# jnvance/DMRG.x

Hardware: NVIDIA B200
Metric: superblock H*psi algorithmic GB/s (higher is better)
Workload: dtype f64

## Files before the change

### dmrg.x_b200/csrc/dev_cuda.cu

```cuda
#include <cuda_runtime.h>
#include <dlfcn.h>
#include <nccl.h>

#include <chrono>
#include <map>
#include <unordered_map>
#include <cstdio>
#include <cstring>
#include <algorithm>
#include <stdexcept>
#include <string>
#include <vector>

#include "dev.h"

namespace dev {

static thread_local std::string g_err;
static long long g_launches = 0;
const char* last_error() { return g_err.c_str(); }
long long launch_count() { return g_launches; }

#define CUDA_OK(call)                                                                                   \
    do {                                                                                                \
        cudaError_t e_ = (call);                                                                        \
        if (e_ != cudaSuccess) {                                                                        \
            char buf_[512];                                                                             \
            snprintf(buf_, sizeof buf_, "%s failed at %s:%d: %s", #call, __FILE__, __LINE__, cudaGetErrorString(e_)); \
            g_err = buf_;                                                                               \
            fprintf(stderr, "[dmrgx] %s\n", buf_);                                                      \
            throw std::runtime_error(buf_);                                                             \
        }                                                                                               \
    } while (0)

struct Stream {
    int device = 0;
    cudaStream_t s = nullptr;
    bool own = false;
    double* partials = nullptr;
    unsigned int* ticket = nullptr;
    int num_sms = 148;
    struct Arena { char* base = nullptr; size_t size = 0; std::map<size_t, size_t> free;  };
    std::vector<Arena> arenas;
    std::unordered_map<void*, size_t> live;
    size_t bytes_reserved = 0, bytes_free = 0, bytes_live = 0, bytes_live_peak = 0;
    double malloc_seconds = 0;
    long long malloc_calls = 0;
    ncclComm_t comm = nullptr;
    int rank = 0, world = 1;
    int spmm_smem = 0;
    bool chain_cfg = false;
    bool gram_cfg = false;
    bool gram_rect_cfg = false;
    cudaStream_t aux = nullptr;
    cudaEvent_t ev_fork = nullptr, ev_join = nullptr;
};

constexpr int RED_BLOCKS = 592;
constexpr int RED_MAXVEC = 40;

int init(int device, void* user_stream, Stream** out) {
    try {
        int ndev = 0;
        cudaError_t e = cudaGetDeviceCount(&ndev);
        if (e != cudaSuccess || ndev == 0) {
            g_err = std::string("no CUDA device: ") + cudaGetErrorString(e) + " — dmrgx has no CPU path";
            return 100;
        }
        CUDA_OK(cudaSetDevice(device));
        Stream* st = new Stream();
        st->device = device;
        if (user_stream) { st->s = (cudaStream_t)user_stream; st->own = false; }
        else { CUDA_OK(cudaStreamCreateWithFlags(&st->s, cudaStreamNonBlocking)); st->own = true; }
        cudaDeviceProp prop;
        CUDA_OK(cudaGetDeviceProperties(&prop, device));
        st->num_sms = prop.multiProcessorCount;
        CUDA_OK(cudaMalloc(&st->partials, sizeof(double) * RED_BLOCKS * RED_MAXVEC));
        CUDA_OK(cudaMalloc(&st->ticket, sizeof(unsigned int)));
        CUDA_OK(cudaMemset(st->ticket, 0, sizeof(unsigned int)));
        *out = st;
        return 0;
    } catch (const std::exception&) { return 100; }
}

static void comm_destroy_(Stream* st);
void destroy(Stream* st) {
    if (!st) return;
    cudaSetDevice(st->device);
    cudaStreamSynchronize(st->s);
    if (getenv("DMRGX_TRACE") || getenv("DMRGX_ALLOC_STATS"))
        fprintf(stderr, "[trace] allocator: %lld cudaMalloc calls, %.3f s, %.2f GB reserved, peak in use %.2f GB\n", st->malloc_calls, st->malloc_seconds,
                st->bytes_reserved / 1e9, st->bytes_live_peak / 1e9);
    if (st->comm) comm_destroy_(st);
    if (st->aux) cudaStreamDestroy(st->aux);
    if (st->ev_fork) cudaEventDestroy(st->ev_fork);
    if (st->ev_join) cudaEventDestroy(st->ev_join);
    for (auto& ar : st->arenas) cudaFree(ar.base);
    cudaFree(st->partials);
    cudaFree(st->ticket);
    if (st->own) cudaStreamDestroy(st->s);
    delete st;
}
void make_current(Stream* st) { cudaSetDevice(st->device); }

constexpr size_t HEAP_SLAB = (size_t)1 << 30, HEAP_GRAIN = (size_t)256 << 20;
static void heap_add_arena(Stream* st, void* slab, size_t sz) {
    Stream::Arena ar; ar.base = (char*)slab; ar.size = sz; ar.free[0] = sz;
    st->arenas.push_back(ar); st->bytes_reserved += sz; st->bytes_free += sz;
}
void* malloc_bytes(Stream* st, size_t bytes) {
    const size_t need = (std::max<size_t>(bytes, 1) + 511) & ~(size_t)511;
    for (;;) {
        Stream::Arena* best_a = nullptr;
        std::map<size_t, size_t>::iterator best;
        size_t best_len = ~(size_t)0;
        for (auto& ar : st->arenas)
            for (auto f = ar.free.begin(); f != ar.free.end(); ++f)
                if (f->second >= need && f->second < best_len) { best_a = &ar; best = f; best_len = f->second; if (best_len == need) break; }
        if (best_a) {
            const size_t off = best->first, len = best->second;
            best_a->free.erase(best);
            if (len > need) best_a->free[off + need] = len - need;
            void* p = best_a->base + off;
            st->live[p] = need;
            st->bytes_free -= need; st->bytes_live += need;
            if (st->bytes_live > st->bytes_live_peak) st->bytes_live_peak = st->bytes_live;
            return p;
        }
        const size_t quarter = std::min(HEAP_SLAB * 8, st->bytes_reserved / 4 / HEAP_GRAIN * HEAP_GRAIN);
        const size_t sz = std::max(std::max(HEAP_SLAB, quarter), (need + HEAP_GRAIN - 1) / HEAP_GRAIN * HEAP_GRAIN);
        void* slab = nullptr;
        const auto t0 = std::chrono::steady_clock::now();
        cudaError_t e = cudaMalloc(&slab, sz);
        if (e != cudaSuccess) {
            cudaGetLastError();
            CUDA_OK(cudaStreamSynchronize(st->s));
            for (size_t i = 0; i < st->arenas.size();) {
                Stream::Arena& ar = st->arenas[i];
                if (ar.free.size() == 1 && ar.free.begin()->second == ar.size) {
                    cudaFree(ar.base); st->bytes_reserved -= ar.size; st->bytes_free -= ar.size; st->arenas.erase(st->arenas.begin() + (long)i);
                } else ++i;
            }
            e = cudaMalloc(&slab, need);
            if (e == cudaSuccess) heap_add_arena(st, slab, need);
        } else heap_add_arena(st, slab, sz);
        st->malloc_seconds += std::chrono::duration<double>(std::chrono::steady_clock::now() - t0).count();
        st->malloc_calls++;
        CUDA_OK(e);
    }
}
void free_bytes(Stream* st, void* p) {
    if (!p) return;
    auto f = st->live.find(p);
    if (f == st->live.end()) return;
    size_t len = f->second;
    st->live.erase(f);
    st->bytes_free += len; st->bytes_live -= len;
    for (auto& ar : st->arenas) {
        if ((char*)p < ar.base || (char*)p >= ar.base + ar.size) continue;
        size_t off = (size_t)((char*)p - ar.base);
        auto nx = ar.free.lower_bound(off);
        if (nx != ar.free.end() && off + len == nx->first) { len += nx->second; nx = ar.free.erase(nx); }
        if (nx != ar.free.begin()) {
            auto pv = std::prev(nx);
            if (pv->first + pv->second == off) { pv->second += len; return; }
        }
        ar.free[off] = len;
        return;
    }
}
void h2d(Stream* st, void* dst, const void* src, size_t bytes) { if (bytes) CUDA_OK(cudaMemcpyAsync(dst, src, bytes, cudaMemcpyHostToDevice, st->s)); }
void d2h(Stream* st, void* dst, const void* src, size_t bytes) { if (bytes) CUDA_OK(cudaMemcpyAsync(dst, src, bytes, cudaMemcpyDeviceToHost, st->s)); }
void d2d(Stream* st, void* dst, const void* src, size_t bytes) { if (bytes) CUDA_OK(cudaMemcpyAsync(dst, src, bytes, cudaMemcpyDeviceToDevice, st->s)); }
void memset0(Stream* st, void* dst, size_t bytes) { if (bytes) CUDA_OK(cudaMemsetAsync(dst, 0, bytes, st->s)); }
void sync(Stream* st) { CUDA_OK(cudaStreamSynchronize(st->s)); }

#define LAUNCH_CHECK() do { ++g_launches; CUDA_OK(cudaGetLastError()); } while (0)

constexpr int BM = 64, BK = 16, NTHREADS = 128;
constexpr int S_MK = BK + 4;
constexpr int S_KM = BM + 4;
constexpr int SMEM_TILE = (BM * S_MK > BK * S_KM) ? BM * S_MK : BK * S_KM;

__device__ __forceinline__ void cp_async8(double* smem_dst, const double* gsrc, bool valid) {
    unsigned s = (unsigned)__cvta_generic_to_shared(smem_dst);
    int sz = valid ? 8 : 0;
    asm volatile("cp.async.ca.shared.global [%0], [%1], 8, %2;\n" ::"r"(s), "l"(gsrc), "r"(sz));
}
__device__ __forceinline__ void cp_async8_all(double* smem_dst, const double* gsrc) {
    unsigned s = (unsigned)__cvta_generic_to_shared(smem_dst);
    asm volatile("cp.async.ca.shared.global [%0], [%1], 8;\n" ::"r"(s), "l"(gsrc));
}
__device__ __forceinline__ void cp_async_commit() { asm volatile("cp.async.commit_group;\n" ::); }
template <int N>
__device__ __forceinline__ void cp_async_wait() { asm volatile("cp.async.wait_group %0;\n" ::"n"(N)); }

__device__ __forceinline__ void dmma_m8n8k4(double& c0, double& c1, double a, double b) {
    asm volatile("mma.sync.aligned.m8n8k4.row.col.f64.f64.f64.f64 {%0,%1}, {%2}, {%3}, {%0,%1};\n"
                 : "+d"(c0), "+d"(c1)
                 : "d"(a), "d"(b));
}

template <bool MK>
struct Stager {
    const double* base;
    int off[8];
    long long kstep;
    int soff;
    int k0;
    unsigned rowmask;
    static constexpr int SI = MK ? 8 * S_MK : 2 * S_KM;
    __device__ __forceinline__ void init(const double* b, long long ld_row, long long ld_k, int ext, int tid) {
        base = b;
        if (MK) {
            const int k = tid & 15, r0 = tid >> 4;
            rowmask = 0;
#pragma unroll
            for (int i = 0; i < 8; ++i) {
                int r = r0 + 8 * i;
                if (r < ext) rowmask |= 1u << i;
                r = r < ext ? r : ext - 1;
                off[i] = (int)(r * ld_row + k * ld_k);
            }
            soff = r0 * S_MK + k;
            k0 = k;
        } else {
            const int r = tid & 63, kk = tid >> 6;
            const int rc = r < ext ? r : ext - 1;
            rowmask = r < ext ? 0xffu : 0u;
#pragma unroll
            for (int i = 0; i < 8; ++i) off[i] = (int)(rc * ld_row + (kk + 2 * i) * ld_k);
            soff = kk * S_KM + r;
            k0 = kk;
        }
        kstep = (long long)BK * ld_k;
    }
    template <bool ALLROWS>
    __device__ __forceinline__ void issue(double* sm, int krem) {
        if (krem >= BK) {
#pragma unroll
            for (int i = 0; i < 8; ++i)
                if (ALLROWS || ((rowmask >> i) & 1u)) cp_async8_all(sm + soff + i * SI, base + off[i]);
        } else {
#pragma unroll
            for (int i = 0; i < 8; ++i) {
                const bool v = (MK ? k0 : k0 + 2 * i) < krem;
                if (ALLROWS || ((rowmask >> i) & 1u)) cp_async8(sm + soff + i * SI, v ? base + off[i] : base, v);
            }
        }
        base += kstep;
    }
};

template <bool A_MK, bool B_NK, bool UNIT, int NMI, int NNI, int NKK = BK / 4>
__device__ __forceinline__ void chunk_mma(double (&acc)[4][4][2], const double* as, const double* bs, double coef) {
    constexpr int a_sm = A_MK ? S_MK : 1, a_sk = A_MK ? 1 : S_KM;
    constexpr int b_sn = B_NK ? S_MK : 1, b_sk = B_NK ? 1 : S_KM;
#pragma unroll
    for (int kk = 0; kk < NKK; ++kk) {
        double a[NMI], b[NNI];
#pragma unroll
        for (int mi = 0; mi < NMI; ++mi) a[mi] = as[mi * 8 * a_sm + kk * 4 * a_sk];
#pragma unroll
        for (int ni = 0; ni < NNI; ++ni) b[ni] = UNIT ? bs[ni * 8 * b_sn + kk * 4 * b_sk] : bs[ni * 8 * b_sn + kk * 4 * b_sk] * coef;
#pragma unroll
        for (int ni = 0; ni < NNI; ++ni)
#pragma unroll
            for (int mi = 0; mi < NMI; ++mi) dmma_m8n8k4(acc[mi][ni][0], acc[mi][ni][1], a[mi], b[ni]);
    }
}

template <int NSTAGE, bool A_MK, bool B_NK, bool FULL, bool UNIT>
__device__ __forceinline__ void gemm_segment(double (&acc)[4][4][2], const Segment& sg, const WorkItem& it, double* As, double* Bs,
                                             int tid, int rbase, int cbase, int g, int t, int nmi, int nni) {
    Stager<A_MK> sa;
    Stager<B_NK> sb;
    sa.init(sg.A + (long long)it.m0 * sg.lda_m, sg.lda_m, sg.lda_k, it.tm, tid);
    sb.init(sg.B + (long long)it.n0 * sg.ldb_n, sg.ldb_n, sg.ldb_k, it.tn, tid);
    const int K = sg.K;
    const int nchunks = (K + BK - 1) / BK;
    const double coef = sg.coef;
    constexpr int a_sm = A_MK ? S_MK : 1, a_sk = A_MK ? 1 : S_KM;
    constexpr int b_sn = B_NK ? S_MK : 1, b_sk = B_NK ? 1 : S_KM;
    const int a_base = (rbase + g) * a_sm + t * a_sk;
    const int b_base = (cbase + g) * b_sn + t * b_sk;
    __syncthreads();
#pragma unroll
    for (int p = 0; p < NSTAGE - 1; ++p) {
        if (p < nchunks) {
            sa.template issue<FULL>(As + p * SMEM_TILE, K - p * BK);
            sb.template issue<FULL>(Bs + p * SMEM_TILE, K - p * BK);
        }
        cp_async_commit();
    }
    int cur = 0, nxt = NSTAGE - 1;
    for (int c = 0; c < nchunks; ++c) {
        if (c + NSTAGE - 1 < nchunks) {
            const int krem = K - (c + NSTAGE - 1) * BK;
            sa.template issue<FULL>(As + nxt * SMEM_TILE, krem);
            sb.template issue<FULL>(Bs + nxt * SMEM_TILE, krem);
        }
        cp_async_commit();
        cp_async_wait<NSTAGE - 1>();
        __syncthreads();
        const double* as = As + cur * SMEM_TILE + a_base;
        const double* bs = Bs + cur * SMEM_TILE + b_base;
        if (FULL) {
            const int krem = K - c * BK;
            if (krem > 12) chunk_mma<A_MK, B_NK, UNIT, 4, 4, 4>(acc, as, bs, coef);
            else if (krem > 8) chunk_mma<A_MK, B_NK, UNIT, 4, 4, 3>(acc, as, bs, coef);
            else if (krem > 4) chunk_mma<A_MK, B_NK, UNIT, 4, 4, 2>(acc, as, bs, coef);
            else chunk_mma<A_MK, B_NK, UNIT, 4, 4, 1>(acc, as, bs, coef);
        } else {
#define MMA_CASE(M_, N_) case (M_) * 5 + (N_): chunk_mma<A_MK, B_NK, UNIT, M_, N_>(acc, as, bs, coef); break;
            switch (nmi * 5 + nni) {
                MMA_CASE(4, 4) MMA_CASE(4, 3) MMA_CASE(4, 2) MMA_CASE(4, 1)
                MMA_CASE(3, 4) MMA_CASE(3, 3) MMA_CASE(3, 2) MMA_CASE(3, 1)
                MMA_CASE(2, 4) MMA_CASE(2, 3) MMA_CASE(2, 2) MMA_CASE(2, 1)
                MMA_CASE(1, 4) MMA_CASE(1, 3) MMA_CASE(1, 2) MMA_CASE(1, 1)
                default: break;
            }
#undef MMA_CASE
        }
        __syncthreads();
        cur = cur + 1 == NSTAGE ? 0 : cur + 1;
        nxt = nxt + 1 == NSTAGE ? 0 : nxt + 1;
    }
}

template <int NSTAGE, bool A_MK, bool B_NK>
__device__ __forceinline__ void gemm_dispatch(double (&acc)[4][4][2], const Segment& sg, const WorkItem& it, double* As, double* Bs,
                                              int tid, int rbase, int cbase, int g, int t, int nmi, int nni) {
    if (sg.coef == 1.0) {
        if (it.tm == BM && it.tn == BM) gemm_segment<NSTAGE, A_MK, B_NK, true, true>(acc, sg, it, As, Bs, tid, rbase, cbase, g, t, 4, 4);
        else gemm_segment<NSTAGE, A_MK, B_NK, false, true>(acc, sg, it, As, Bs, tid, rbase, cbase, g, t, nmi, nni);
    } else gemm_segment<NSTAGE, A_MK, B_NK, false, false>(acc, sg, it, As, Bs, tid, rbase, cbase, g, t, nmi, nni);
}

template <int NSTAGE>
__global__ void __launch_bounds__(NTHREADS, 3) chain_kernel(const WorkItem* __restrict__ items, const Segment* __restrict__ segs,
                                                            const double* __restrict__ xbase, double* __restrict__ ybase,
                                                            double* __restrict__ wbase) {
    extern __shared__ __align__(16) double chain_smem[];
    double* As = chain_smem;
    double* Bs = chain_smem + NSTAGE * SMEM_TILE;
    WorkItem it = items[blockIdx.x];
    if (it.c_in_y) it.C = (double*)((char*)(it.c_in_y == 1 ? ybase : wbase) + (size_t)it.C);
    const int tid = threadIdx.x;
    const int warp = tid >> 5, lane = tid & 31;
    const int wm = warp >> 1, wn = warp & 1;
    const int g = lane >> 2, t = lane & 3;
    const int tm = it.tm, tn = it.tn;
    const int hm = ((tm + 15) >> 4) << 3, hn = ((tn + 15) >> 4) << 3;
    const int rbase = wm * hm, cbase = wn * hn;
    int nmi = (tm - rbase + 7) / 8; nmi = nmi < 0 ? 0 : (nmi > (hm >> 3) ? (hm >> 3) : nmi);
    int nni = (tn - cbase + 7) / 8; nni = nni < 0 ? 0 : (nni > (hn >> 3) ? (hn >> 3) : nni);

    double acc[4][4][2];
#pragma unroll
    for (int mi = 0; mi < 4; ++mi)
#pragma unroll
        for (int ni = 0; ni < 4; ++ni) { acc[mi][ni][0] = 0.0; acc[mi][ni][1] = 0.0; }

    for (int s = it.seg_begin; s < it.seg_end; ++s) {
        Segment sg = segs[s];
        if (sg.flags & SEGF_A_X) sg.A = (const double*)((const char*)xbase + (size_t)sg.A);
        if (sg.flags & SEGF_B_X) sg.B = (const double*)((const char*)xbase + (size_t)sg.B);
        if (sg.type == SEG_GEMM) {
            const bool a_mk = (sg.lda_k == 1) || (sg.lda_m != 1);
            const bool b_nk = (sg.ldb_k == 1) || (sg.ldb_n != 1);
            if (a_mk) {
                if (b_nk) gemm_dispatch<NSTAGE, true, true>(acc, sg, it, As, Bs, tid, rbase, cbase, g, t, nmi, nni);
                else gemm_dispatch<NSTAGE, true, false>(acc, sg, it, As, Bs, tid, rbase, cbase, g, t, nmi, nni);
            } else {
                if (b_nk) gemm_dispatch<NSTAGE, false, true>(acc, sg, it, As, Bs, tid, rbase, cbase, g, t, nmi, nni);
                else gemm_dispatch<NSTAGE, false, false>(acc, sg, it, As, Bs, tid, rbase, cbase, g, t, nmi, nni);
            }
        } else if (sg.type == SEG_AXPY) {
            const double* base = sg.A + (long long)(it.m0 + rbase + g) * sg.lda_m + (long long)(it.n0 + cbase + 2 * t) * sg.lda_k;
            const long long sm8 = 8 * sg.lda_m, sn8 = 8 * sg.lda_k, sn1 = sg.lda_k;
            double v[4][4][2];
#pragma unroll
            for (int mi = 0; mi < 4; ++mi) {
                const bool rok = mi < nmi && rbase + mi * 8 + g < tm;
#pragma unroll
                for (int ni = 0; ni < 4; ++ni) {
                    const int col = cbase + ni * 8 + 2 * t;
                    const bool c0 = rok && ni < nni && col < tn, c1 = rok && ni < nni && col + 1 < tn;
                    const double* q = base + mi * sm8 + ni * sn8;
                    v[mi][ni][0] = c0 ? q[0] : 0.0;
                    v[mi][ni][1] = c1 ? q[sn1] : 0.0;
                }
            }
            const double coef = sg.coef;
#pragma unroll
            for (int mi = 0; mi < 4; ++mi)
#pragma unroll
                for (int ni = 0; ni < 4; ++ni) { acc[mi][ni][0] += coef * v[mi][ni][0]; acc[mi][ni][1] += coef * v[mi][ni][1]; }
        } else if (sg.type == SEG_CSRA) {
            const double* xb = sg.A + (long long)(it.n0 + cbase + 2 * t) * sg.ldb_n;
#pragma unroll
            for (int mi = 0; mi < 4; ++mi) {
                const int row = rbase + mi * 8 + g;
                if (mi >= nmi || row >= tm) continue;
                const int r = sg.row0 + it.m0 + row;
                const int e1 = sg.rowptr[r + 1];
                for (int e = sg.rowptr[r]; e < e1; ++e) {
                    const double v = sg.B[e] * sg.coef;
                    const double* xr = xb + (long long)sg.colidx[e] * sg.ldb_k;
#pragma unroll
                    for (int ni = 0; ni < 4; ++ni) {
                        const int col = cbase + ni * 8 + 2 * t;
                        if (ni < nni && col < tn) acc[mi][ni][0] += v * xr[(long long)(ni * 8) * sg.ldb_n];
                        if (ni < nni && col + 1 < tn) acc[mi][ni][1] += v * xr[(long long)(ni * 8 + 1) * sg.ldb_n];
                    }
                }
            }
        } else if (sg.type == SEG_CSRB) {
            const double* vb = sg.A + (long long)(it.m0 + rbase + g) * sg.lda_m;
#pragma unroll
            for (int ni = 0; ni < 4; ++ni) {
#pragma unroll
                for (int h = 0; h < 2; ++h) {
                    const int col = cbase + ni * 8 + 2 * t + h;
                    if (ni >= nni || col >= tn) continue;
                    const int r = sg.row0 + it.n0 + col;
                    const int e1 = sg.rowptr[r + 1];
                    for (int e = sg.rowptr[r]; e < e1; ++e) {
                        const double v = sg.B[e] * sg.coef;
                        const double* vc = vb + (long long)sg.colidx[e] * sg.lda_k;
#pragma unroll
                        for (int mi = 0; mi < 4; ++mi)
                            if (mi < nmi && rbase + mi * 8 + g < tm) acc[mi][ni][h] += v * vc[(long long)(mi * 8) * sg.lda_m];
                    }
                }
            }
        } else if (sg.type == SEG_CSRADD) {
#pragma unroll
            for (int mi = 0; mi < 4; ++mi) {
                const int row = rbase + mi * 8 + g;
                if (mi >= nmi || row >= tm) continue;
                const int r = sg.row0 + it.m0 + row;
                const int e1 = sg.rowptr[r + 1];
                for (int e = sg.rowptr[r]; e < e1; ++e) {
                    const int lc = sg.colidx[e] - sg.d - it.n0 - cbase - 2 * t;
                    const double v = sg.B[e] * sg.coef;
#pragma unroll
                    for (int ni = 0; ni < 4; ++ni) {
                        const int col = cbase + ni * 8 + 2 * t;
                        if (ni < nni && lc == ni * 8 && col < tn) acc[mi][ni][0] += v;
                        if (ni < nni && lc == ni * 8 + 1 && col + 1 < tn) acc[mi][ni][1] += v;
                    }
                }
            }
        } else if (sg.type == SEG_DIAG) {
#pragma unroll
            for (int mi = 0; mi < 4; ++mi) {
                const int row = rbase + mi * 8 + g;
                if (mi >= nmi || row >= tm) continue;
#pragma unroll
                for (int ni = 0; ni < 4; ++ni)
#pragma unroll
                    for (int h = 0; h < 2; ++h) {
                        const int col = cbase + ni * 8 + 2 * t + h;
                        if (ni < nni && col < tn && it.m0 + row + sg.d == it.n0 + col) acc[mi][ni][h] += sg.coef;
                    }
            }
        }
    }
#pragma unroll
    for (int mi = 0; mi < 4; ++mi) {
        const int row = rbase + mi * 8 + g;
        if (mi >= nmi || row >= tm) continue;
#pragma unroll
        for (int ni = 0; ni < 4; ++ni) {
#pragma unroll
            for (int h = 0; h < 2; ++h) {
                const int col = cbase + ni * 8 + 2 * t + h;
                if (ni >= nni || col >= tn) continue;
                double* p = it.C + (long long)row * it.ldc + col;
                if (it.mode == 0) *p = acc[mi][ni][h];
                else atomicAdd(p, acc[mi][ni][h]);
            }
        }
    }
}

void run_chain(Stream* st, const WorkItem* d_items, int nitems, const Segment* d_segs, const double* x, double* y, double* w) {
    if (nitems <= 0) return;
    constexpr int smem2 = 2 * 2 * SMEM_TILE * (int)sizeof(double), smem3 = 2 * 3 * SMEM_TILE * (int)sizeof(double);
    if (!st->chain_cfg) {
        CUDA_OK(cudaFuncSetAttribute(chain_kernel<3>, cudaFuncAttributeMaxDynamicSharedMemorySize, smem3));
        st->chain_cfg = true;
    }
    constexpr int deep_below = 1800;
    if (nitems < deep_below) chain_kernel<3><<<nitems, NTHREADS, smem3, st->s>>>(d_items, d_segs, x, y, w);
    else chain_kernel<2><<<nitems, NTHREADS, smem2, st->s>>>(d_items, d_segs, x, y, w);
    LAUNCH_CHECK();
}

constexpr int SP_BD = 256, SP_CH = 4, SP_AMAX = 24, SP_BMAX = 8;

__device__ __forceinline__ unsigned smem_u32(const void* p) { return (unsigned)__cvta_generic_to_shared(p); }
__device__ __forceinline__ void mbar_init(unsigned long long* b, int count) {
    asm volatile("mbarrier.init.shared::cta.b64 [%0], %1;\n" ::"r"(smem_u32(b)), "r"(count));
    asm volatile("fence.mbarrier_init.release.cluster;\n" ::: "memory");
}
__device__ __forceinline__ void mbar_expect_tx(unsigned long long* b, unsigned bytes) {
    asm volatile("mbarrier.arrive.expect_tx.shared::cta.b64 _, [%0], %1;\n" ::"r"(smem_u32(b)), "r"(bytes) : "memory");
}
__device__ __forceinline__ void bulk_g2s(void* dst, const void* src, unsigned bytes, unsigned long long* b) {
    asm volatile("cp.async.bulk.shared::cluster.global.mbarrier::complete_tx::bytes [%0], [%1], %2, [%3];\n" ::"r"(smem_u32(dst)), "l"(src), "r"(bytes),
                 "r"(smem_u32(b))
                 : "memory");
}
__device__ __forceinline__ void mbar_wait(unsigned long long* b, unsigned parity) {
    unsigned ok;
    do {
        asm volatile("{\n.reg .pred p;\nmbarrier.try_wait.parity.shared::cta.b64 p, [%1], %2;\nselp.u32 %0, 1, 0, p;\n}\n" : "=r"(ok) : "r"(smem_u32(b)), "r"(parity) : "memory");
    } while (!ok);
}

template <class T>
__device__ __forceinline__ void sp_stage(T* dst, const T* src, int count, int tid) {
    for (int i = tid; i < count * (int)(sizeof(T) / 8); i += SP_BD) ((double*)dst)[i] = __ldg((const double*)src + i);
}

__global__ void __launch_bounds__(SP_BD, 3) spmm_kernel(const SpTile* __restrict__ tiles, const SpASlot* __restrict__ aslots, const SpSSlot* __restrict__ sslots,
                                                       const SpBSlot* __restrict__ bslots, const double* __restrict__ x, double* __restrict__ y) {
    extern __shared__ __align__(16) unsigned char sp_smem[];
    __shared__ unsigned long long mbar;
    __shared__ SpTile s_tile;
    __shared__ SpASlot s_a[SP_AMAX];
    __shared__ SpSSlot s_s[SP_AMAX];
    __shared__ SpBSlot s_b[SP_BMAX];
    const int tid = threadIdx.x;
    if (tid < (int)(sizeof(SpTile) / 4)) ((int*)&s_tile)[tid] = ((const int*)(tiles + blockIdx.x))[tid];
    if (tid == 0) mbar_init(&mbar, 1);
    __syncthreads();
    const int nR = s_tile.nR, nrows = s_tile.nrows;
    const long long off0 = s_tile.off;
    const double* src0 = x + off0;
    const int cnt = nrows * nR;
    const int head = (int)(((unsigned long long)src0 >> 3) & 1ull);
    double* xs = (double*)sp_smem + head;
    const int bulk = (cnt - head) & ~1;
    if (tid == 0 && bulk > 0) {
        mbar_expect_tx(&mbar, (unsigned)bulk * 8u);
        bulk_g2s(xs + head, src0 + head, (unsigned)bulk * 8u, &mbar);
    }
    if (tid == 32 && head) xs[0] = src0[0];
    if (tid == 64 && head + bulk < cnt) xs[cnt - 1] = src0[cnt - 1];
    const int na = s_tile.a_count, ns = s_tile.s_count, nb = s_tile.b_count;
    bool staged = false;

    for (int cb0 = 0; cb0 < nR; cb0 += SP_CH * SP_BD) {
        double acc[SP_CH][SP_ROWS];
#pragma unroll
        for (int j = 0; j < SP_CH; ++j)
#pragma unroll
            for (int r = 0; r < SP_ROWS; ++r) acc[j][r] = 0.0;
        const int c0 = cb0 + tid;
        bool cok[SP_CH];
#pragma unroll
        for (int j = 0; j < SP_CH; ++j) cok[j] = c0 + j * SP_BD < nR;

        for (int a0 = 0; a0 < na; a0 += SP_AMAX) {
            const int nbatch = min(SP_AMAX, na - a0);
            __syncthreads();
            sp_stage(s_a, aslots + s_tile.a_begin + a0, nbatch, tid);
            __syncthreads();
            for (int k = 0; k < nbatch; ++k) {
#pragma unroll
                for (int h = 0; h < SP_ROWS; h += 4) {
                    double v[4][SP_CH];
#pragma unroll
                    for (int r = 0; r < 4; ++r) {
                        const double* p = x + s_a[k].src[h + r] + c0;
#pragma unroll
                        for (int j = 0; j < SP_CH; ++j) v[r][j] = cok[j] ? __ldg(p + j * SP_BD) : 0.0;
                    }
#pragma unroll
                    for (int r = 0; r < 4; ++r) {
                        const double w = s_a[k].w[h + r];
#pragma unroll
                        for (int j = 0; j < SP_CH; ++j) acc[j][h + r] += w * v[r][j];
                    }
                }
            }
        }
        if (!staged) { if (bulk > 0) mbar_wait(&mbar, 0); staged = true; }
        for (int a0 = 0; a0 < ns; a0 += SP_AMAX) {
            const int nbatch = min(SP_AMAX, ns - a0);
            __syncthreads();
            sp_stage(s_s, sslots + s_tile.s_begin + a0, nbatch, tid);
            __syncthreads();
            for (int k = 0; k < nbatch; ++k) {
#pragma unroll
                for (int r = 0; r < SP_ROWS; ++r) {
                    const double* p = xs + s_s[k].roff[r] + c0;
                    const double w = s_s[k].w[r];
#pragma unroll
                    for (int j = 0; j < SP_CH; ++j)
                        if (cok[j]) acc[j][r] += w * p[j * SP_BD];
                }
            }
        }
        for (int b0 = 0; b0 < nb; b0 += SP_BMAX) {
            const int nbatch = min(SP_BMAX, nb - b0);
            __syncthreads();
            sp_stage(s_b, bslots + s_tile.b_begin + b0, nbatch, tid);
            __syncthreads();
            for (int k = 0; k < nbatch; ++k) {
                const int W = s_b[k].W, ld = s_b[k].ld;
                const int* ecol = s_b[k].ecol + c0;
                const double* eval = s_b[k].eval + c0;
                if (s_b[k].all_in) {
#pragma unroll
                    for (int h = 0; h < SP_ROWS; h += 4) {
                        int roff[4];
                        double w[4];
#pragma unroll
                        for (int r = 0; r < 4; ++r) { roff[r] = s_b[k].roff[h + r]; w[r] = s_b[k].w[h + r]; }
                        for (int t = 0; t < W; ++t) {
                            int cf[SP_CH];
                            double vb[SP_CH];
#pragma unroll
                            for (int j = 0; j < SP_CH; ++j) {
                                cf[j] = cok[j] ? __ldg(ecol + t * ld + j * SP_BD) : 0;
                                vb[j] = cok[j] ? __ldg(eval + t * ld + j * SP_BD) : 0.0;
                            }
#pragma unroll
                            for (int j = 0; j < SP_CH; ++j) {
                                if (vb[j] == 0.0) continue;
#pragma unroll
                                for (int r = 0; r < 4; ++r) acc[j][h + r] += (w[r] * vb[j]) * xs[roff[r] + cf[j]];
                            }
                        }
                    }
                } else {
#pragma unroll
                    for (int h = 0; h < SP_ROWS; h += 4) {
                        const double* gx[4];
                        double w[4];
#pragma unroll
                        for (int r = 0; r < 4; ++r) { gx[r] = x + s_b[k].src[h + r]; w[r] = s_b[k].w[h + r]; }
                        for (int t = 0; t < W; ++t) {
                            int cf[SP_CH];
                            double vb[SP_CH];
#pragma unroll
                            for (int j = 0; j < SP_CH; ++j) {
                                cf[j] = cok[j] ? __ldg(ecol + t * ld + j * SP_BD) : 0;
                                vb[j] = cok[j] ? __ldg(eval + t * ld + j * SP_BD) : 0.0;
                            }
#pragma unroll
                            for (int j = 0; j < SP_CH; ++j) {
                                if (vb[j] == 0.0) continue;
#pragma unroll
                                for (int r = 0; r < 4; ++r) acc[j][h + r] += (w[r] * vb[j]) * __ldg(gx[r] + cf[j]);
                            }
                        }
                    }
                }
            }
        }
#pragma unroll
        for (int r = 0; r < SP_ROWS; ++r) {
            if (r >= nrows) continue;
            double* yr = y + off0 + (long long)r * nR + c0;
#pragma unroll
            for (int j = 0; j < SP_CH; ++j)
                if (cok[j]) yr[j * SP_BD] = acc[j][r];
        }
    }
}

void run_spmm(Stream* st, const SpTile* d_tiles, int ntiles, const SpASlot* d_aslots, const SpSSlot* d_sslots, const SpBSlot* d_bslots, const double* x, double* y,
              int max_nR) {
    if (ntiles <= 0) return;
    if (max_nR > SP_MAX_NR) throw std::runtime_error("run_spmm: right sector too wide for the shared-memory stage");
    const int smem = SP_ROWS * max_nR * 8 + 32;
    if (smem > st->spmm_smem) {
        CUDA_OK(cudaFuncSetAttribute(spmm_kernel, cudaFuncAttributeMaxDynamicSharedMemorySize, smem));
        st->spmm_smem = smem;
    }
    spmm_kernel<<<ntiles, SP_BD, smem, st->s>>>(d_tiles, d_aslots, d_sslots, d_bslots, x, y);
    LAUNCH_CHECK();
}

__global__ void __launch_bounds__(256) reduce_kernel(const ReduceItem* __restrict__ items, double* __restrict__ ybase, const double* __restrict__ wbase) {
    const ReduceItem it = items[blockIdx.x];
    double* dst = it.dst_in_y ? (double*)((char*)ybase + (size_t)it.dst) : it.dst;
    const double* src = (const double*)((const char*)wbase + it.src_off);
    const int cnt = it.tm * it.tn;
    for (int e = threadIdx.x; e < cnt; e += blockDim.x) {
        double v = src[e];
        for (int p = 1; p < it.nparts; ++p) v += src[(long long)p * cnt + e];
        dst[(long long)(e / it.tn) * it.ldc + (e % it.tn)] = v;
    }
}
void run_reduce(Stream* st, const ReduceItem* d_items, int nitems, double* y, const double* w) {
    if (nitems <= 0) return;
    reduce_kernel<<<nitems, 256, 0, st->s>>>(d_items, y, w);
    LAUNCH_CHECK();
}

__device__ __forceinline__ double warp_sum(double v) {
#pragma unroll
    for (int o = 16; o > 0; o >>= 1) v += __shfl_xor_sync(0xffffffffu, v, o);
    return v;
}

__device__ __forceinline__ unsigned long long splitmix64(unsigned long long z) {
    z += 0x9E3779B97F4A7C15ULL;
    z = (z ^ (z >> 30)) * 0xBF58476D1CE4E5B9ULL;
    z = (z ^ (z >> 27)) * 0x94D049BB133111EBULL;
    return z ^ (z >> 31);
}
__global__ void fill_random_kernel(double* x, long long n, unsigned long long seed, long long first) {
    for (long long i = blockIdx.x * (long long)blockDim.x + threadIdx.x; i < n; i += (long long)gridDim.x * blockDim.x)
        x[i] = (double)(splitmix64(seed + (unsigned long long)(first + i) * 0x9E3779B97F4A7C15ULL) >> 11) / 9007199254740992.0 - 0.5;
}
void fill_random(Stream* st, double* x, long long n, unsigned long long seed, long long first) {
    if (n <= 0) return;
    int blocks = (int)std::min<long long>((n + 255) / 256, RED_BLOCKS);
    fill_random_kernel<<<blocks, 256, 0, st->s>>>(x, n, seed, first);
    LAUNCH_CHECK();
}

template <int NV>
__global__ void __launch_bounds__(256) gs_pass_kernel(const double* __restrict__ V, long long ldv, int nvec, double* __restrict__ w, long long n,
                                                      const double* __restrict__ coef, double* __restrict__ dots, double* __restrict__ nrm2,
                                                      double* __restrict__ partials, unsigned int* __restrict__ ticket) {
    __shared__ double c[NV];
    __shared__ double sh[NV + 1][8];
    __shared__ bool last;
    if (threadIdx.x < NV) c[threadIdx.x] = (coef && threadIdx.x < nvec) ? coef[threadIdx.x] : 0.0;
    __syncthreads();
    double s[NV + 1];
#pragma unroll
    for (int i = 0; i <= NV; ++i) s[i] = 0.0;
    for (long long q = blockIdx.x * (long long)blockDim.x + threadIdx.x; q < n; q += (long long)gridDim.x * blockDim.x) {
        double v[NV];
#pragma unroll
        for (int i = 0; i < NV; ++i) v[i] = i < nvec ? V[i * ldv + q] : 0.0;
        double wq = w[q];
        if (coef) {
#pragma unroll
            for (int i = 0; i < NV; ++i) wq -= c[i] * v[i];
            w[q] = wq;
        }
        if (dots) {
#pragma unroll
            for (int i = 0; i < NV; ++i) s[i] += v[i] * wq;
        }
        s[NV] += wq * wq;
    }
    const int lane = threadIdx.x & 31, wid = threadIdx.x >> 5;
#pragma unroll
    for (int i = 0; i <= NV; ++i) {
        const double r = warp_sum(s[i]);
        if (lane == 0) sh[i][wid] = r;
    }
    __syncthreads();
    if (threadIdx.x <= NV) {
        double r = 0.0;
        for (int k = 0; k < 8; ++k) r += sh[threadIdx.x][k];
        partials[(long long)blockIdx.x * (NV + 1) + threadIdx.x] = r;
    }
    __threadfence();
    __syncthreads();
    if (threadIdx.x == 0) last = atomicAdd(ticket, 1u) == gridDim.x - 1;
    __syncthreads();
    if (!last) return;
    __threadfence();
    for (int i = wid; i <= NV; i += 8) {
        double r = 0.0;
        for (int b = lane; b < (int)gridDim.x; b += 32) r += partials[(long long)b * (NV + 1) + i];
        r = warp_sum(r);
        if (lane == 0) {
            if (i < NV) { if (dots && i < nvec) dots[i] = r; }
            else if (nrm2) *nrm2 = r;
// ... 1067 lines not shown
```

Baseline: 65.18.

## Add stacked warp geometry for tall or wide partial tiles in chain GEMM

Adds alternative warp layouts (rows or columns stacked) for partial tiles where one dimension is full and the other between half and nearly full. Each warp then covers a 16-wide strip with 5-7 fragments instead of leaving some warps idle in the 2x2 grid. It also folds the coefficient into the MMA operands, widens the fast FULL path to near-full tiles, and replaces the unrolled K-remainder variants with a trimmed loop. The cost is extra register mapping complexity, a block-wide sync to check segment types, and more template instantiations.

```diff
diff --git a/dmrg.x_b200/csrc/dev_cuda.cu b/dmrg.x_b200/csrc/dev_cuda.cu
--- a/dmrg.x_b200/csrc/dev_cuda.cu
+++ b/dmrg.x_b200/csrc/dev_cuda.cu
@@ -252,12 +252,16 @@
     }
 };
 
-template <bool A_MK, bool B_NK, bool UNIT, int NMI, int NNI, int NKK = BK / 4>
-__device__ __forceinline__ void chunk_mma(double (&acc)[4][4][2], const double* as, const double* bs, double coef) {
+enum : int { GEO_GRID = 0, GEO_ROWS = 1, GEO_COLS = 2 };
+constexpr int SEL_STACK = 25;
+
+template <bool A_MK, bool B_NK, bool UNIT, int NMI, int NNI, bool TRIM = false>
+__device__ __forceinline__ void chunk_mma(double (&acc)[4][4][2], const double* as, const double* bs, double coef, int krem = BK) {
     constexpr int a_sm = A_MK ? S_MK : 1, a_sk = A_MK ? 1 : S_KM;
     constexpr int b_sn = B_NK ? S_MK : 1, b_sk = B_NK ? 1 : S_KM;
 #pragma unroll
-    for (int kk = 0; kk < NKK; ++kk) {
+    for (int kk = 0; kk < BK / 4; ++kk) {
+        if (TRIM && kk > 0 && krem <= 4 * kk) break;
         double a[NMI], b[NNI];
 #pragma unroll
         for (int mi = 0; mi < NMI; ++mi) a[mi] = as[mi * 8 * a_sm + kk * 4 * a_sk];
@@ -270,9 +274,31 @@
     }
 }
 
-template <int NSTAGE, bool A_MK, bool B_NK, bool FULL, bool UNIT>
+template <bool A_MK, bool B_NK, bool ROWS, int F>
+__device__ __forceinline__ void chunk_mma_stack(double (&acc)[4][4][2], const double* as, const double* bs, double coef) {
+    constexpr int a_sm = A_MK ? S_MK : 1, a_sk = A_MK ? 1 : S_KM;
+    constexpr int b_sn = B_NK ? S_MK : 1, b_sk = B_NK ? 1 : S_KM;
+    constexpr int NM = ROWS ? 2 : F, NN = ROWS ? F : 2;
+#pragma unroll
+    for (int kk = 0; kk < BK / 4; ++kk) {
+        double a[NM], b[NN];
+#pragma unroll
+        for (int mi = 0; mi < NM; ++mi) a[mi] = ROWS ? as[mi * 8 * a_sm + kk * 4 * a_sk] * coef : as[mi * 8 * a_sm + kk * 4 * a_sk];
+#pragma unroll
+        for (int ni = 0; ni < NN; ++ni) b[ni] = ROWS ? bs[ni * 8 * b_sn + kk * 4 * b_sk] : bs[ni * 8 * b_sn + kk * 4 * b_sk] * coef;
+#pragma unroll
+        for (int ni = 0; ni < NN; ++ni)
+#pragma unroll
+            for (int mi = 0; mi < NM; ++mi) {
+                double* c = ROWS ? acc[2 * (ni >> 2) + mi][ni & 3] : acc[mi & 3][2 * (mi >> 2) + ni];
+                dmma_m8n8k4(c[0], c[1], a[mi], b[ni]);
+            }
+    }
+}
+
+template <int NSTAGE, bool A_MK, bool B_NK, bool FULL>
 __device__ __forceinline__ void gemm_segment(double (&acc)[4][4][2], const Segment& sg, const WorkItem& it, double* As, double* Bs,
-                                             int tid, int rbase, int cbase, int g, int t, int nmi, int nni) {
+                                             int tid, int rbase, int cbase, int g, int t, int sel) {
     Stager<A_MK> sa;
     Stager<B_NK> sb;
     sa.init(sg.A + (long long)it.m0 * sg.lda_m, sg.lda_m, sg.lda_k, it.tm, tid);
@@ -305,21 +331,23 @@
         __syncthreads();
         const double* as = As + cur * SMEM_TILE + a_base;
         const double* bs = Bs + cur * SMEM_TILE + b_base;
-        if (FULL) {
+        if constexpr (FULL) {
             const int krem = K - c * BK;
-            if (krem > 12) chunk_mma<A_MK, B_NK, UNIT, 4, 4, 4>(acc, as, bs, coef);
-            else if (krem > 8) chunk_mma<A_MK, B_NK, UNIT, 4, 4, 3>(acc, as, bs, coef);
-            else if (krem > 4) chunk_mma<A_MK, B_NK, UNIT, 4, 4, 2>(acc, as, bs, coef);
-            else chunk_mma<A_MK, B_NK, UNIT, 4, 4, 1>(acc, as, bs, coef);
+            if (krem >= BK) chunk_mma<A_MK, B_NK, true, 4, 4>(acc, as, bs, coef);
+            else chunk_mma<A_MK, B_NK, true, 4, 4, true>(acc, as, bs, coef, krem);
         } else {
-#define MMA_CASE(M_, N_) case (M_) * 5 + (N_): chunk_mma<A_MK, B_NK, UNIT, M_, N_>(acc, as, bs, coef); break;
-            switch (nmi * 5 + nni) {
+#define MMA_CASE(M_, N_) case (M_) * 5 + (N_): chunk_mma<A_MK, B_NK, false, M_, N_>(acc, as, bs, coef); break;
+#define STACK_CASE(R_, F_) case SEL_STACK + 3 * !(R_) + (F_) - 5: chunk_mma_stack<A_MK, B_NK, R_, F_>(acc, as, bs, coef); break;
+            switch (sel) {
                 MMA_CASE(4, 4) MMA_CASE(4, 3) MMA_CASE(4, 2) MMA_CASE(4, 1)
                 MMA_CASE(3, 4) MMA_CASE(3, 3) MMA_CASE(3, 2) MMA_CASE(3, 1)
                 MMA_CASE(2, 4) MMA_CASE(2, 3) MMA_CASE(2, 2) MMA_CASE(2, 1)
                 MMA_CASE(1, 4) MMA_CASE(1, 3) MMA_CASE(1, 2) MMA_CASE(1, 1)
+                STACK_CASE(true, 5) STACK_CASE(true, 6) STACK_CASE(true, 7)
+                STACK_CASE(false, 5) STACK_CASE(false, 6) STACK_CASE(false, 7)
                 default: break;
             }
+#undef STACK_CASE
 #undef MMA_CASE
         }
         __syncthreads();
@@ -330,11 +358,9 @@
 
 template <int NSTAGE, bool A_MK, bool B_NK>
 __device__ __forceinline__ void gemm_dispatch(double (&acc)[4][4][2], const Segment& sg, const WorkItem& it, double* As, double* Bs,
-                                              int tid, int rbase, int cbase, int g, int t, int nmi, int nni) {
-    if (sg.coef == 1.0) {
-        if (it.tm == BM && it.tn == BM) gemm_segment<NSTAGE, A_MK, B_NK, true, true>(acc, sg, it, As, Bs, tid, rbase, cbase, g, t, 4, 4);
-        else gemm_segment<NSTAGE, A_MK, B_NK, false, true>(acc, sg, it, As, Bs, tid, rbase, cbase, g, t, nmi, nni);
-    } else gemm_segment<NSTAGE, A_MK, B_NK, false, false>(acc, sg, it, As, Bs, tid, rbase, cbase, g, t, nmi, nni);
+                                              int tid, int rbase, int cbase, int g, int t, int sel) {
+    if (it.tm > BM - 8 && it.tn > BM - 8 && sg.coef == 1.0) gemm_segment<NSTAGE, A_MK, B_NK, true>(acc, sg, it, As, Bs, tid, rbase, cbase, g, t, sel);
+    else gemm_segment<NSTAGE, A_MK, B_NK, false>(acc, sg, it, As, Bs, tid, rbase, cbase, g, t, sel);
 }
 
 template <int NSTAGE>
@@ -352,9 +378,26 @@
     const int g = lane >> 2, t = lane & 3;
     const int tm = it.tm, tn = it.tn;
     const int hm = ((tm + 15) >> 4) << 3, hn = ((tn + 15) >> 4) << 3;
-    const int rbase = wm * hm, cbase = wn * hn;
+    int rbase = wm * hm, cbase = wn * hn;
     int nmi = (tm - rbase + 7) / 8; nmi = nmi < 0 ? 0 : (nmi > (hm >> 3) ? (hm >> 3) : nmi);
     int nni = (tn - cbase + 7) / 8; nni = nni < 0 ? 0 : (nni > (hn >> 3) ? (hn >> 3) : nni);
+    int geo = GEO_GRID;
+    if (tm > BM - 8 && tn > BM / 2 && tn <= BM - 8) geo = GEO_ROWS;
+    else if (tn > BM - 8 && tm > BM / 2 && tm <= BM - 8) geo = GEO_COLS;
+    if (geo != GEO_GRID) {
+        int slow = 0;
+        for (int s = it.seg_begin + tid; s < it.seg_end; s += NTHREADS) slow |= segs[s].type != SEG_GEMM;
+        if (__syncthreads_or(slow)) geo = GEO_GRID;
+    }
+    int sel = nmi * 5 + nni;
+    if (geo != GEO_GRID) {
+        rbase = geo == GEO_ROWS ? 16 * warp : 0;
+        cbase = geo == GEO_COLS ? 16 * warp : 0;
+        nmi = nni = 4;
+        sel = SEL_STACK + 3 * (geo == GEO_COLS) + (((geo == GEO_ROWS ? tn : tm) + 7) >> 3) - 5;
+    }
+    const int mmask = geo == GEO_ROWS ? 1 : 3, nmask = geo == GEO_COLS ? 1 : 3;
+    const int rsplit = geo == GEO_COLS ? 32 : 0, csplit = geo == GEO_ROWS ? 32 : 0;
 
     double acc[4][4][2];
 #pragma unroll
@@ -370,11 +413,11 @@
             const bool a_mk = (sg.lda_k == 1) || (sg.lda_m != 1);
             const bool b_nk = (sg.ldb_k == 1) || (sg.ldb_n != 1);
             if (a_mk) {
-                if (b_nk) gemm_dispatch<NSTAGE, true, true>(acc, sg, it, As, Bs, tid, rbase, cbase, g, t, nmi, nni);
-                else gemm_dispatch<NSTAGE, true, false>(acc, sg, it, As, Bs, tid, rbase, cbase, g, t, nmi, nni);
+                if (b_nk) gemm_dispatch<NSTAGE, true, true>(acc, sg, it, As, Bs, tid, rbase, cbase, g, t, sel);
+                else gemm_dispatch<NSTAGE, true, false>(acc, sg, it, As, Bs, tid, rbase, cbase, g, t, sel);
             } else {
-                if (b_nk) gemm_dispatch<NSTAGE, false, true>(acc, sg, it, As, Bs, tid, rbase, cbase, g, t, nmi, nni);
-                else gemm_dispatch<NSTAGE, false, false>(acc, sg, it, As, Bs, tid, rbase, cbase, g, t, nmi, nni);
+                if (b_nk) gemm_dispatch<NSTAGE, false, true>(acc, sg, it, As, Bs, tid, rbase, cbase, g, t, sel);
+                else gemm_dispatch<NSTAGE, false, false>(acc, sg, it, As, Bs, tid, rbase, cbase, g, t, sel);
             }
         } else if (sg.type == SEG_AXPY) {
             const double* base = sg.A + (long long)(it.m0 + rbase + g) * sg.lda_m + (long long)(it.n0 + cbase + 2 * t) * sg.lda_k;
@@ -470,14 +513,14 @@
     }
 #pragma unroll
     for (int mi = 0; mi < 4; ++mi) {
-        const int row = rbase + mi * 8 + g;
-        if (mi >= nmi || row >= tm) continue;
+        if (mi >= nmi) continue;
 #pragma unroll
         for (int ni = 0; ni < 4; ++ni) {
+            const int row = rbase + 8 * (mi & mmask) + rsplit * (ni >> 1) + g;
 #pragma unroll
             for (int h = 0; h < 2; ++h) {
-                const int col = cbase + ni * 8 + 2 * t + h;
-                if (ni >= nni || col >= tn) continue;
+                const int col = cbase + 8 * (ni & nmask) + csplit * (mi >> 1) + 2 * t + h;
+                if (ni >= nni || row >= tm || col >= tn) continue;
                 double* p = it.C + (long long)row * it.ldc + col;
                 if (it.mode == 0) *p = acc[mi][ni][h];
                 else atomicAdd(p, acc[mi][ni][h]);
```

After: 62.40 (median of 6 runs). 0.957x the previous value.
